# codeMonkey339/Congestion-control-with-BitTorren

Hardware: AMD Instinct MI355X
Metric: GiB/s device-resident SHA-1 over 512KB chunks; % of HBM-read roofline (higher is better)
Workload: dtype u32; 1 GPU; 4096 x 524288 B chunks per GPU, device-resident (BASELINE config 2); chunks_per_gpu=4096, chunk_bytes=524288, kernel=split_u4_2prod, kernel_requested=auto, streams=1, parallelism=chunk-sharded x1, no collective

## Files before the change

congestion-control-with-bittorren_amd/csrc/sha1_kernels.h:

```cpp
#pragma once

#include <hip/hip_runtime.h>
#include <stdint.h>

struct BatchArgs {
    const uint8_t* base;
    const uint64_t* off;
    const uint32_t* len;
    uint32_t ulen;
    uint32_t n;
    const uint32_t* order;
    uint8_t* dig;
    const uint32_t* init_state;
    uint64_t prefix_bytes;
    uint32_t* out_state;
    const uint32_t* plan;
};

enum LaunchCounter {
    kLaunchLane, kLaunchFused, kLaunchSplit1, kLaunchSplit4, kLaunchSplit11Lane, kLaunchSplit11Shared,
    kLaunchQuad, kLaunchStudy, kLaunchMixed, kLaunchSort, kLaunchDrain, kLaunchCounters
};
void count_launch(LaunchCounter which);

hipError_t launch_lane(const BatchArgs& A, hipStream_t st);
hipError_t launch_fused(const BatchArgs& A, hipStream_t st);
constexpr int kSplitUnitQuad = 416;
bool split_unit_built(int unit_blocks);
hipError_t launch_split(const BatchArgs& A, int unit_blocks, hipStream_t st);
bool split_unit_study_built(int unit_blocks);
hipError_t launch_split_study(const BatchArgs& A, int unit_blocks, hipStream_t st);
uint32_t mixed_grid(uint32_t groups, int cus, uint32_t* hcap);
constexpr uint32_t kBigExact = 4096;
struct BigFix {
    const uint32_t* cnt;
    uint32_t tiles;
    const uint32_t* len;
    const uint32_t* id;
    uint32_t* order;
    uint32_t* sorted_len;
};
hipError_t launch_mixed(const BatchArgs& A, const uint32_t* sorted_len, const BigFix* big, uint32_t* plan, int cus,
                        const int* forced, hipStream_t st);
hipError_t launch_plan_layout(const BatchArgs& A, const uint32_t* sorted_len, const BigFix* big, uint32_t* plan,
                              hipStream_t st);
struct VqDrainArgs {
    const uint8_t* data;
    const uint64_t* off;
    const uint32_t* len;
    const uint8_t* exp;
    const uint32_t* grp;
    const uint32_t* pub;
    const uint32_t* stop;
    uint8_t* alive;
    uint8_t* res;
    uint32_t* done;
    uint32_t* last_done;
    uint8_t* dig;
    uint32_t* claim;
    uint32_t grp_ring;
    uint32_t pad;
    uint64_t idle_ticks;
    uint64_t life_ticks;
};
hipError_t launch_vq_drain(const VqDrainArgs& Q, uint32_t grid, hipStream_t st);

struct PvEntry {
    uint32_t session;
    uint32_t from;
    uint32_t upto;
    uint32_t len;
    uint32_t final;
    uint32_t gen;
    uint32_t pad[2];
};
struct PvArgs {
    const uint8_t* data;
    uint64_t stride;
    const PvEntry* work;
    uint32_t n;
    uint32_t sessions;
    uint32_t* state;
    const uint32_t* expected;
    uint32_t* result;
    uint32_t* done;
    const uint8_t* dummy;
};
hipError_t launch_progress(const PvArgs& P, int depth, hipStream_t st);
hipError_t launch_progress_shared(const PvArgs& P, hipStream_t st);

struct UpdateArgs {
    uint8_t* ctx;
    uint64_t n_contexts;
    const uint32_t* index;
    uint32_t n;
    const uint8_t* base;
    const uint64_t* off;
    const uint32_t* len;
    uint64_t* mid_off;
    uint32_t* mid_len;
    uint32_t* state;
    uint8_t* dig;
};
hipError_t launch_update_init(const UpdateArgs& U, hipStream_t st);
hipError_t launch_update_pre(const UpdateArgs& U, hipStream_t st);
hipError_t launch_update_post(const UpdateArgs& U, hipStream_t st);
hipError_t launch_update_final(const UpdateArgs& U, hipStream_t st);

struct GatherArgs {
    const uint8_t* base;
// ... 44 lines not shown
```

congestion-control-with-bittorren_amd/csrc/sha1_kernels.hip:

```cpp
#include <hip/hip_runtime.h>
#include <stdint.h>

#include <algorithm>
#include <cstdlib>
#include <cstring>

#include "sha1_fused.hpp"
#include "sha1_split.hpp"

#define PLAN_SPLIT4 0.743
#define PLAN_SPLIT8 0.860
#define PLAN_FUSED4T 1.254
#define PLAN_FUSED4S 1.334
#define PLAN_FUSED8T 2.502
#define PLAN_FUSED8S 2.628
#define PLAN_FUSED_SHARE 0.955

__global__ __launch_bounds__(256) void sha1_lane_kernel(BatchArgs A) {
    const uint32_t e = blockIdx.x * blockDim.x + threadIdx.x;
    if (e >= A.n) return;
    const Entry en = fetch_entry(A, e);
    uint32_t h[5];
    load_init(A, en.id, h);
    lane_blocks(A, en, 0, h);
// ... 781 lines not shown
        for (uint32_t m = 32; m >= 1; m >>= 1) key = min(key, (uint64_t)__shfl_xor(key, m));
        if (lane == 0u) red[wv] = key;
    }
    __syncthreads();
    if (t == 0) {
        ts[5] = __builtin_amdgcn_s_memrealtime();
        cs[5] = __builtin_amdgcn_s_memtime();
        uint64_t key = red[0];
#pragma unroll
        for (uint32_t w = 1; w < kMaxCand / 64; ++w) key = min(key, red[w]);
        uint32_t bi = (uint32_t)key;
        if (cmk[2] <= cmk[bi] * 1.005f) bi = 2;
        plan[0] = cmode[bi];
        plan[1] = cmode[bi] == 1 ? 0u : chead[bi];
        plan[2] = cmode[bi] == 1 ? 0u : cf[bi];
#pragma unroll
        for (int i = 1; i < 6; ++i) plan[7 + i] = static_cast<uint32_t>(ts[i] - ts[0]);
#pragma unroll
        for (int i = 1; i < 6; ++i) plan[13 + i] = static_cast<uint32_t>(cs[i] - cs[0]);
#pragma unroll
        for (int i = 0; i < 3; ++i) plan[20 + i] = static_cast<uint32_t>(sub[i] - cs[0]);
        plan[23] = nrun;
#pragma unroll
        for (int i = 0; i < 3; ++i) plan[24 + i] = static_cast<uint32_t>(bsub[i] - cs[0]);
        plan[27] = simcyc;
    }
}

__device__ __forceinline__ uint64_t splitmix64(uint64_t x) {
    uint64_t z = x + 0x9E3779B97F4A7C15ull;
    z = (z ^ (z >> 30)) * 0xBF58476D1CE4E5B9ull;
    z = (z ^ (z >> 27)) * 0x94D049BB133111EBull;
    return z ^ (z >> 31);
}

__global__ __launch_bounds__(kSynthThreads) void synth_fill_kernel(uint8_t* dst, const uint64_t* off,
                                                         const uint32_t* lens, uint32_t ulen,
                                                         uint64_t first, uint64_t seed) {
    const uint64_t c = blockIdx.x;
    const uint32_t len = lens ? lens[c] : ulen;
    uint8_t* out = dst + (off ? off[c] : c * (uint64_t)ulen);
    const uint64_t key = seed ^ ((first + c) << 24);
    const uint32_t nw = len >> 3;
    uint64_t* o = reinterpret_cast<uint64_t*>(out);
    for (uint32_t w = threadIdx.x; w < nw; w += blockDim.x) o[w] = splitmix64(key ^ (uint64_t)w);
    const uint32_t rem = len & 7u;
    if (rem && threadIdx.x == 0) {
        const uint64_t v = splitmix64(key ^ (uint64_t)nw);
        for (uint32_t b = 0; b < rem; ++b) out[8ull * nw + b] = (uint8_t)(v >> (8 * b));
    }
}

__global__ __launch_bounds__(256) void compare_kernel(const uint8_t* dig, const uint8_t* exp,
                                                      uint32_t n, uint8_t* mismatch) {
    const uint32_t i = blockIdx.x * blockDim.x + threadIdx.x;
    if (i >= n) return;
    uint32_t diff = 0;
#pragma unroll
    for (int b = 0; b < 20; ++b) diff |= (uint32_t)(dig[20ull * i + b] ^ exp[20ull * i + b]);
    mismatch[i] = diff ? 1 : 0;
}

hipError_t launch_lane(const BatchArgs& A, hipStream_t st) {
    if (A.n == 0) return hipSuccess;
    const uint32_t grid = (A.n + 255u) / 256u;
    count_launch(kLaunchLane);
    hipLaunchKernelGGL(sha1_lane_kernel, dim3(grid), dim3(256), 0, st, A);
    return hipGetLastError();
}

hipError_t launch_fused(const BatchArgs& A, hipStream_t st) {
    if (A.n == 0) return hipSuccess;
    count_launch(kLaunchFused);
    hipLaunchKernelGGL(sha1_fused_kernel, dim3((A.n + 255u) / 256u), dim3(256), 0, st, A);
    return hipGetLastError();
}

__attribute__((weak)) bool split_unit_study_built(int) { return false; }
__attribute__((weak)) hipError_t launch_split_study(const BatchArgs&, int, hipStream_t) {
    return hipErrorInvalidValue;
}

bool split_unit_built(int u) {
    return u == 1 || u == 4 || u == 11 || u == kSplitUnitQuad || split_unit_study_built(u);
}

static_assert(kSplitThreads<1, kSplitV<1>, 1> == 128, "unit 1: consumer + producer");
static_assert(kSplitThreads<1, kSplitV<4>, kSplitNProd<4>> == 256, "unit 4: consumer, two producers, wave 2 empty");
static_assert(kSplitThreads<2, kSplit8V, 2> == 512 && kSplitThreads<2, kSplit8V & ~kVCoop, 2> == 512,
              "unit 11: the 8-wave layout");
static_assert(kSplitThreads<1, kSplitQuadV, 2> == 256, "unit 416: as unit 4");

hipError_t launch_split(const BatchArgs& A, int unit_blocks, hipStream_t st) {
    if (A.n == 0) return hipSuccess;
    const uint32_t groups = (A.n + 63u) / 64u;
    switch (unit_blocks) {
    case 1:
        count_launch(kLaunchSplit1);
        launch_shape<1, 1>(A, groups, st);
        break;
    case 4:
        count_launch(kLaunchSplit4);
        launch_shape<4, 1, kSplitV<4>, kSplitNProd<4>>(A, groups, st);
        break;
    case 11:
        if (A.off == nullptr && A.order == nullptr) {
            count_launch(kLaunchSplit11Lane);
            launch_shape<2, 2, kSplit8V & ~kVCoop, 2>(A, (groups + 1) / 2, st);
        } else {
            count_launch(kLaunchSplit11Shared);
            launch_shape<2, 2, kSplit8V, 2>(A, (groups + 1) / 2, st);
        }
        break;
    case kSplitUnitQuad:
        count_launch(kLaunchQuad);
        launch_shape<4, 1, kSplitQuadV, 2>(A, (A.n + 15u) / 16u, st);
        break;
    default: return launch_split_study(A, unit_blocks, st);
    }
    return hipGetLastError();
}

uint32_t mixed_grid(uint32_t groups, int cus, uint32_t* hcap) {
    *hcap = std::min<uint32_t>(std::min<uint32_t>(groups, 4u * (uint32_t)cus), kPlanMaxH);
    return groups;
}

hipError_t launch_plan_layout(const BatchArgs& A, const uint32_t* sorted_len, const BigFix* big, uint32_t* plan,
                              hipStream_t st) {
    if (A.n == 0) return hipSuccess;
    const uint32_t groups = (A.n + 63u) / 64u;
    const uint32_t words = (groups + 31u) / 32u;
    uint64_t* lay_tb = reinterpret_cast<uint64_t*>(plan + 64);
    uint32_t* lay_bits = reinterpret_cast<uint32_t*>(lay_tb + words);
    uint32_t* lay_blk = lay_bits + words;
    hipLaunchKernelGGL(plan_layout_kernel, dim3(words), dim3(kLayoutThreads), 0, st, A, sorted_len,
                       big ? *big : BigFix{}, lay_tb, lay_bits, lay_blk);
    return hipGetLastError();
}

hipError_t launch_mixed(const BatchArgs& A, const uint32_t* sorted_len, const BigFix* big, uint32_t* plan, int cus,
                        const int* forced, hipStream_t st) {
    if (A.n == 0) return hipSuccess;
    const uint32_t groups = (A.n + 63u) / 64u;
    uint32_t hcap;
    const uint32_t grid = mixed_grid(groups, cus, &hcap);
    const uint32_t words = (groups + 31u) / 32u;
    uint64_t* lay_tb = reinterpret_cast<uint64_t*>(plan + 64);
    uint32_t* lay_bits = reinterpret_cast<uint32_t*>(lay_tb + words);
    const uint32_t* lay_blk = lay_bits + words;
    count_launch(kLaunchMixed);
    if (!forced) {
        const hipError_t le = launch_plan_layout(A, sorted_len, big, plan, st);
        if (le != hipSuccess) return le;
    }
    hipLaunchKernelGGL(plan_mixed_kernel, dim3(1), dim3(kPlanThreads), 0, st, A, sorted_len,
                       (uint32_t)cus, hcap, forced ? 1 : 0, forced ? (uint32_t)forced[0] : 0u,
                       forced ? (uint32_t)forced[1] : 0u, forced ? (uint32_t)forced[2] : 0u, plan, lay_tb,
                       lay_bits, lay_blk);
    hipError_t e = hipGetLastError();
    if (e != hipSuccess) return e;
    BatchArgs B = A;
    B.plan = plan;
    const char* disp = getenv("SHA1CHUNK_MIXED_DISPATCH");
    const bool persistent = !(disp && !strcmp(disp, "hw"));
    if (persistent)
        hipLaunchKernelGGL(sha1_mixed_persistent_kernel, dim3((uint32_t)cus), dim3(kMixedThreads), 0, st, B,
                           plan + 3);
    else
        hipLaunchKernelGGL(sha1_mixed_kernel, dim3(grid), dim3(kMixedThreads), 0, st, B);
    return hipGetLastError();
}

hipError_t launch_vq_drain(const VqDrainArgs& Q, uint32_t grid, hipStream_t st) {
    count_launch(kLaunchDrain);
    hipLaunchKernelGGL(sha1_vq_drain_kernel, dim3(grid), dim3(kMixedThreads), 0, st, Q);
    return hipGetLastError();
}

hipError_t launch_synth(uint8_t* dst, const uint64_t* off, const uint32_t* lens, uint32_t ulen,
                        uint64_t first, uint64_t count, uint64_t seed, hipStream_t st) {
    if (count == 0) return hipSuccess;
    if (count > kSynthMaxChunks) return hipErrorInvalidValue;
    hipLaunchKernelGGL(synth_fill_kernel, dim3((uint32_t)count), dim3(kSynthThreads), 0, st, dst, off, lens,
                       ulen, first, seed);
    return hipGetLastError();
}

hipError_t launch_compare(const uint8_t* dig, const uint8_t* exp, uint32_t n, uint8_t* mismatch,
                          hipStream_t st) {
    if (n == 0) return hipSuccess;
    hipLaunchKernelGGL(compare_kernel, dim3((n + 255u) / 256u), dim3(256), 0, st, dig, exp, n,
                       mismatch);
    return hipGetLastError();
}

#ifdef SHA1CHUNK_CHECKED
extern "C" __attribute__((visibility("default"))) long long s1be_checked_violations(int reset) {
    int cur = 0, nd = 0;
    if (hipGetDevice(&cur) != hipSuccess || hipGetDeviceCount(&nd) != hipSuccess) return -1;
// ... 17 lines not shown
```

congestion-control-with-bittorren_amd/csrc/sha1_runtime.hip:

```cpp
#include <algorithm>
#include <cstdio>
#include <cstdlib>
#include <cstring>
#include <mutex>
#include <numeric>
#include <string>
#include <thread>
#include <vector>

#include "sha1_runtime_internal.h"

using namespace s1rt;

namespace {
int split_unit(size_t n, int cus) {
    if (const char* e = getenv("SHA1CHUNK_SPLIT_UNIT")) return atoi(e);
    if ((n + 15) / 16 <= size_t(std::max(0, cus - drain_cus_held()))) return kSplitUnitQuad;
    const size_t groups = (n + 63) / 64;
    if (groups <= size_t(cus)) return 4;
    if (groups <= size_t(cus) * 2) return 11;
    return 1;
}

hipError_t launch(int kernel, const BatchArgs& A, int cus, hipStream_t st) {
    switch (kernel) {
    case SHA1CHUNK_KERNEL_LANE: return launch_lane(A, st);
    case SHA1CHUNK_KERNEL_FUSED: return launch_fused(A, st);
    case SHA1CHUNK_KERNEL_SPLIT: return launch_split(A, split_unit(A.n, cus), st);
    default: return hipErrorInvalidValue;
    }
}

int check_batch(const BatchArgs& A) {
    if (A.n > 0xffffffffu - 1024u)
        return fail(SHA1CHUNK_EINVAL, "batch of %u chunks: at most 2^32 - 1025 per call", A.n);
    if (A.n > 0 && (reinterpret_cast<uintptr_t>(A.dig) & 3u))
        return fail(SHA1CHUNK_EALIGN, "digest buffer must be 4-byte aligned");
    return SHA1CHUNK_OK;
}
}

namespace s1rt {
int choose_kernel(int kernel, size_t n, int cus) {
    if (kernel != SHA1CHUNK_KERNEL_AUTO) return kernel;
    if (const char* f = getenv("SHA1CHUNK_FORCE_KERNEL")) {
        if (!strcmp(f, "lane")) return SHA1CHUNK_KERNEL_LANE;
        if (!strcmp(f, "fused")) return SHA1CHUNK_KERNEL_FUSED;
        if (!strcmp(f, "split")) return SHA1CHUNK_KERNEL_SPLIT;
    }
    const size_t groups = (n + 63) / 64;
    return groups <= size_t(cus) * 2 ? SHA1CHUNK_KERNEL_SPLIT : SHA1CHUNK_KERNEL_FUSED;
}

int launch_checked(int kernel, const BatchArgs& A, hipStream_t st, int cus) {
    if (kernel < SHA1CHUNK_KERNEL_LANE || kernel > SHA1CHUNK_KERNEL_SPLIT)
        return fail(SHA1CHUNK_EINVAL, "unknown kernel id %d", kernel);
    if (int rc = check_batch(A)) return rc;
    if (kernel == SHA1CHUNK_KERNEL_SPLIT && !split_unit_built(split_unit(A.n, cus)))
        return fail(SHA1CHUNK_EINVAL, "split shape %d is not in this library (A/B shapes: `make ab`)",
                    split_unit(A.n, cus));
    hipError_t e = launch(kernel, A, cus, st);
    if (e != hipSuccess) return fail(SHA1CHUNK_EHIP, "kernel launch: %s", hipGetErrorString(e));
    return SHA1CHUNK_OK;
}

bool use_mixed(size_t n, int cus) {
    if (getenv("SHA1CHUNK_FORCE_KERNEL")) return false;
    const char* e = getenv("SHA1CHUNK_MIXED");
    if (e && !strcmp(e, "0")) return false;
    if (e && !strcmp(e, "all")) return true;
    return (n + 63) / 64 > size_t(cus);
}

int launch_mixed_checked(const BatchArgs& A, const uint32_t* sorted_len, const BigFix* big, uint32_t* plan, int cus,
                         hipStream_t st) {
    if (int rc = check_batch(A)) return rc;
    int forced[3] = {0, 0, 0};
    bool force = false;
    if (const char* e = getenv("SHA1CHUNK_MIXED_PLAN")) {
        uint32_t hcap;
        const uint32_t groups = (A.n + 63u) / 64u;
        (void)mixed_grid(groups, cus, &hcap);
        if (sscanf(e, "%d,%d,%d", &forced[0], &forced[1], &forced[2]) != 3 || forced[0] < 0 ||
            forced[0] > 1 ||
            (forced[0] == 0 && (forced[1] < 0 || ((uint32_t)forced[1] > hcap && (uint32_t)forced[1] != groups) ||
                                (forced[2] != 4 && forced[2] != 8))))
            return fail(SHA1CHUNK_EINVAL,
                        "SHA1CHUNK_MIXED_PLAN=%s: want 0,H,F (0 <= H <= %u or H = %u, F 4|8) or 1,0,0", e,
                        hcap, groups);
        force = true;
    }
    hipError_t e = launch_mixed(A, sorted_len, big, plan, cus, force ? forced : nullptr, st);
    if (e != hipSuccess) return fail(SHA1CHUNK_EHIP, "mixed kernel launch: %s", hipGetErrorString(e));
    if (const char* d = getenv("SHA1CHUNK_MIXED_DEBUG"); d && atoi(d)) {
        uint32_t p[28];
        HIP_TRY(hipMemcpyAsync(p, plan, sizeof p, hipMemcpyDeviceToHost, st));
        HIP_TRY(hipStreamSynchronize(st));
        fprintf(stderr, "sha1chunk mixed plan: n=%u groups=%u cus=%d mode=%u H=%u F=%u\n", A.n,
                (A.n + 63u) / 64u, cus, p[0], p[1], p[2]);
        if (!force && p[12])
            fprintf(stderr,
                    "sha1chunk mixed planner stages: scan %.1f bounds %.1f sweep %.1f pass2 %.1f pass3 %.1f us;"
// ... 470 lines not shown
```

congestion-control-with-bittorren_amd/csrc/sha1_split.hpp:

```cpp
#ifndef SHA1_SPLIT_HPP
#define SHA1_SPLIT_HPP

#include "sha1_lane.hpp"

constexpr int kWBlockBytes = 20 * 1024;

constexpr int kVWK = 1;
constexpr int kVUnmask = 4;
constexpr int kVRead10 = 8;
constexpr int kVSkipWave2 = 64;
constexpr int kVLayout8 = 128;
constexpr int kVCross = 256;
constexpr int kVProbe = 2048;
constexpr int kVCoop = 8192;
constexpr int kVQuad = 8192 * 4;

template <int U>
constexpr int kSplitV = U == 4 ? (kVWK | kVUnmask | kVSkipWave2 | kVRead10 | kVCoop)
                               : U == 3 ? kVUnmask : (kVWK | kVUnmask);
template <int U>
constexpr int kSplitNProd = U == 4 ? 2 : 1;
constexpr int kSplit8V = kVWK | kVUnmask | kVLayout8 | kVCross | kVCoop;
constexpr int kSplitQuadV = kVWK | kVUnmask | kVSkipWave2 | kVCoop | kVQuad;
template <int PAIRS, int V, int NPROD>
constexpr int kSplitThreads = (V & kVLayout8) ? 512 : 64 * PAIRS * (1 + NPROD) + ((V & kVSkipWave2) ? 64 : 0);


__device__ __forceinline__ void split_barrier() {
    __builtin_amdgcn_s_waitcnt(0xC07F);
    asm volatile("s_barrier" ::: "memory");
}

__device__ __forceinline__ void split_barrier_timed(uint64_t& acc) {
    __builtin_amdgcn_s_waitcnt(0xC07F);
    const uint64_t t0 = __builtin_amdgcn_s_memtime();
    asm volatile("s_barrier" ::: "memory");
    acc += __builtin_amdgcn_s_memtime() - t0;
}

template <int T, bool WK>
struct SchedWrite {
    __device__ __forceinline__ static void run(uint32_t (&w)[16], uint8_t* slot, int lane) {
        if constexpr (T < 80) {
            if constexpr (T >= 16) sched_step<T>(w);
            if constexpr ((T & 3) == 3) {
                constexpr int j = (T - 3) & 15;
                constexpr uint32_t k = WK ? round_k<T>() : 0u;
                *reinterpret_cast<uint4*>(slot + (T >> 2) * 1024 + lane * 16) =
                    make_uint4(w[j] + k, w[j + 1] + k, w[j + 2] + k, w[j + 3] + k);
            }
            SchedWrite<T + 1, WK>::run(w, slot, lane);
        }
    }
};

__device__ __forceinline__ uint32_t total_blocks(uint32_t len) {
    return (len >> 6) + (((len & 63u) < 56u) ? 1u : 2u);
}

__device__ __forceinline__ void tail_block_words(const Entry& en, uint32_t k, uint32_t (&w)[16]) {
    const uint32_t nfull = en.len >> 6, rem = en.len & 63u;
    const uint64_t bits = (uint64_t)en.len * 8ull;
    if (k < nfull) {
        load_block16(en.p + 64ull * k, w);
#pragma unroll
        for (int j = 0; j < 16; ++j) w[j] = bswap(w[j]);
    } else if (k == nfull) {
        if (rem) {
            load_block_partial(en.p + 64ull * k, rem, w);
        } else {
#pragma unroll
            for (int j = 0; j < 16; ++j) w[j] = 0u;
        }
#pragma unroll
        for (int j = 0; j < 16; ++j) w[j] = pad_word(bswap(w[j]), j, (int)rem);
        if (rem < 56u) {
            w[14] = (uint32_t)(bits >> 32);
            w[15] = (uint32_t)bits;
        }
    } else {
#pragma unroll
        for (int j = 0; j < 14; ++j) w[j] = 0u;
        w[14] = (uint32_t)(bits >> 32);
        w[15] = (uint32_t)bits;
    }
}

template <int U, bool WK, int NPROD = 1>
__device__ __forceinline__ void produce_block(uint32_t k, uint32_t (&w)[16], uint8_t* ring, int lane,
                                              uint64_t* bw = nullptr) {
    const uint32_t m = k / U, j = k - m * U;
    SchedWrite<0, WK>::run(w, ring + ((m & 1u) * U + j) * kWBlockBytes, lane);
    if (NPROD == 1 ? j == U - 1 : (U == NPROD || (k & 1u) == 1u)) {
        if (bw)
            split_barrier_timed(*bw);
        else
            split_barrier();
    }
}


template <int U, bool WK, int NPROD = 1>
__device__ __forceinline__ void produce_stage(const Entry& en, uint32_t s, uint32_t S, Stage& cur,
                                              uint8_t* ring, int lane) {
#pragma unroll
    for (int half = 0; half < 2; ++half) {
// ... 70 lines not shown
template <bool MASK>
__device__ __forceinline__ void commit(uint32_t (&h)[5], const uint32_t (&v)[5], bool live) {
    if constexpr (MASK) {
#pragma unroll
        for (int i = 0; i < 5; ++i) h[i] = live ? h[i] + v[i] : h[i];
    } else {
#pragma unroll
        for (int i = 0; i < 5; ++i) h[i] += v[i];
    }
}

__device__ __forceinline__ void probe_store(const BatchArgs& A, uint32_t row, uint64_t waited, uint64_t total,
                                            uint32_t blocks) {
    uint32_t* o = reinterpret_cast<uint32_t*>(A.dig + 20ull * row);
    o[0] = (uint32_t)waited;
    o[1] = (uint32_t)(waited >> 32);
    o[2] = (uint32_t)total;
    o[3] = (uint32_t)(total >> 32);
    o[4] = blocks;
}

template <int B, int NB, bool WK>
struct BurstRounds {
    __device__ __forceinline__ static void run(uint32_t (&v)[5], const uint32_t (&Wc)[80], uint32_t (&Wn)[80],
                                               const uint8_t* slot) {
        if constexpr (B < NB) {
            __builtin_amdgcn_sched_barrier(0);
            read_w_groups<4 * B / NB, 4 * (B + 1) / NB>(slot, Wn);
            __builtin_amdgcn_sched_barrier(0);
            RoundsW<80 * B / NB, 80 * (B + 1) / NB, WK>::run(v, Wc);
            BurstRounds<B + 1, NB, WK>::run(v, Wc, Wn, slot);
        }
    }
};

template <int U, int J, int V, bool MASK>
__device__ __forceinline__ void consume_block(uint32_t k, uint32_t T, uint32_t (&h)[5],
                                              const uint32_t (&Wc)[80], uint32_t (&Wn)[80],
                                              const uint8_t* ring, int lane, uint64_t& bw) {
    constexpr int jn = (J + 1) % U;
    constexpr int slot_idx = (((J + 1) / U) & 1) * U + jn;
    const uint8_t* slot = ring + slot_idx * kWBlockBytes + lane * 16;
    uint32_t v[5] = {h[0], h[1], h[2], h[3], h[4]};
    if constexpr (jn == 0) split_barrier_or_timed<V>(bw);
    BurstRounds<0, (V & kVRead10) ? 2 : 4, (V & kVWK) != 0>::run(v, Wc, Wn, slot);
    commit<MASK>(h, v, k < T);
}

template <int U, int J, int V, bool MASK>
struct ConsumeUnits {
    __device__ __forceinline__ static void run(uint32_t k0, uint32_t T, uint32_t (&h)[5],
                                               uint32_t (&Wa)[80], uint32_t (&Wb)[80],
                                               const uint8_t* ring, int lane, uint64_t& bw) {
        if constexpr (J < 2 * U) {
            consume_block<U, J, V, MASK>(k0 + J, T, h, Wa, Wb, ring, lane, bw);
            ConsumeUnits<U, J + 1, V, MASK>::run(k0, T, h, Wb, Wa, ring, lane, bw);
        }
    }
};

template <int U, int V>
__device__ __forceinline__ void consume_all(const BatchArgs& A, const Entry& en, bool valid, uint32_t T,
                                            uint32_t units, const uint8_t* ring, int lane) {
    uint32_t h[5];
    load_init(A, en.id, h);
    uint32_t Wa[80], Wb[80];
    split_barrier();
    read_w_groups<0, 4>(ring + lane * 16, Wa);
    const uint32_t Tmin = __builtin_amdgcn_readfirstlane(wave_min(valid ? T : 0xffffffffu));
    const uint32_t full = (V & kVUnmask) ? min(Tmin, units * U) / (2 * U) * (2 * U) : 0u;
    uint32_t k = 0;
    uint64_t bw = 0;
    const uint64_t t0 = (V & kVProbe) ? __builtin_amdgcn_s_memtime() : 0;
    for (; k < full; k += 2 * U) ConsumeUnits<U, 0, V, false>::run(k, T, h, Wa, Wb, ring, lane, bw);
    for (; k < units * U; k += 2 * U) ConsumeUnits<U, 0, V, true>::run(k, T, h, Wa, Wb, ring, lane, bw);
    if constexpr ((V & kVProbe) != 0) {
        const uint64_t tot = __builtin_amdgcn_s_memtime() - t0;
        if (lane == 0) probe_store(A, en.id & ~63u, bw, tot, units * U);
        return;
    }
    if (valid) emit(A, en.id, h);
}

constexpr int kQuadBlockBytes = 5 * 1024;

template <int SEL>
__device__ __forceinline__ uint32_t quad_bcast(uint32_t x) {
    return (uint32_t)__builtin_amdgcn_update_dpp(0, (int)x, SEL * 0x55, 0xf, 0xf, true);
}

__device__ __forceinline__ void quad_align() { asm volatile(".p2align 3"); }

template <int T, int END>
struct RoundsQ {
    __device__ __forceinline__ static void run(uint32_t (&v)[5], const uint32_t (&W)[20]) {
        if constexpr (T < END) {
            round_step<T, true, true>(v, quad_bcast<(T >> 2) & 3>(W[4 * (T >> 4) + (T & 3)]));
            RoundsQ<T + 1, END>::run(v, W);
        }
    }
};

__device__ __forceinline__ void quad_read_w(const uint8_t* slot, uint32_t (&W)[20]) {
#pragma unroll
    for (int q = 0; q < 5; ++q) unpack4(W + 4 * q, *reinterpret_cast<const uint4*>(slot + q * 1024));
}

template <int U, int J, int V, bool MASK>
__device__ __forceinline__ void quad_consume_block(uint32_t k, uint32_t T, uint32_t (&h)[5],
                                                   const uint32_t (&Wc)[20], uint32_t (&Wn)[20],
                                                   const uint8_t* ring, int lane, uint64_t& bw) {
    constexpr int jn = (J + 1) % U;
    constexpr int slot_idx = (((J + 1) / U) & 1) * U + jn;
    const uint8_t* slot = ring + slot_idx * kQuadBlockBytes + lane * 16;
    uint32_t v[5] = {h[0], h[1], h[2], h[3], h[4]};
    if constexpr (jn == 0) split_barrier_or_timed<V>(bw);
    __builtin_amdgcn_sched_barrier(0);
    quad_read_w(slot, Wn);
    __builtin_amdgcn_sched_barrier(0);
    quad_align();
    __builtin_amdgcn_sched_barrier(0);
    RoundsQ<0, 80>::run(v, Wc);
    __builtin_amdgcn_sched_barrier(0);
    __builtin_amdgcn_s_waitcnt(0xC07F);
    __builtin_amdgcn_sched_barrier(0);
    commit<MASK>(h, v, k < T);
    __builtin_amdgcn_sched_barrier(0);
}

template <int U, int J, int V, bool MASK>
struct QuadConsumeUnits {
    __device__ __forceinline__ static void run(uint32_t k0, uint32_t T, uint32_t (&h)[5], uint32_t (&Wa)[20],
                                               uint32_t (&Wb)[20], const uint8_t* ring, int lane, uint64_t& bw) {
        if constexpr (J < 2 * U) {
            quad_consume_block<U, J, V, MASK>(k0 + J, T, h, Wa, Wb, ring, lane, bw);
            QuadConsumeUnits<U, J + 1, V, MASK>::run(k0, T, h, Wb, Wa, ring, lane, bw);
        }
    }
};

template <int T>
struct QuadSchedWrite {
    __device__ __forceinline__ static void run(uint32_t (&w)[16], uint8_t* slot, bool j1, bool j2,
                                               const uint32_t (&kq)[5]) {
        if constexpr (T < 80) {
            if constexpr (T >= 16) sched_step<T>(w);
            if constexpr ((T & 15) == 15) {
                constexpr int q = T >> 4;
                uint32_t o[4];
#pragma unroll
                for (int i = 0; i < 4; ++i) {
                    const uint32_t lo = j1 ? w[4 + i] : w[i], hi = j1 ? w[12 + i] : w[8 + i];
                    o[i] = (j2 ? hi : lo) + kq[q];
                }
                *reinterpret_cast<uint4*>(slot + q * 1024) = make_uint4(o[0], o[1], o[2], o[3]);
            }
            QuadSchedWrite<T + 1>::run(w, slot, j1, j2, kq);
        }
    }
};

template <int U>
__device__ __forceinline__ void quad_produce_block(uint32_t k, uint32_t (&w)[16], uint8_t* ring, int lane,
                                                   const uint32_t (&kq)[5]) {
    const uint32_t m = k / U, j = k - m * U;
    QuadSchedWrite<0>::run(w, ring + ((m & 1u) * U + j) * kQuadBlockBytes + lane * 16, (lane & 1) != 0,
                           (lane & 2) != 0, kq);
    if ((k & 1u) == 1u && ((k >> 1) % (U / 2)) + 2 >= U / 2) split_barrier();
}

__device__ __forceinline__ void quad_block_words(const uint32_t (&x)[4], uint32_t (&w)[16]) {
    uint32_t y[4];
#pragma unroll
    for (int i = 0; i < 4; ++i) y[i] = bswap(x[i]);
#pragma unroll
    for (int i = 0; i < 4; ++i) {
        w[i] = quad_bcast<0>(y[i]);
        w[4 + i] = quad_bcast<1>(y[i]);
        w[8 + i] = quad_bcast<2>(y[i]);
        w[12 + i] = quad_bcast<3>(y[i]);
    }
}

__device__ __forceinline__ void quad_load_stage(const u32x4u* src, uint32_t s, uint32_t (&x)[8]) {
#pragma unroll
    for (int b = 0; b < 2; ++b) unpack4(x + 4 * b, src[8u * s + 4u * b]);
}

template <int U>
__device__ __forceinline__ void quad_produce_stage(const u32x4u* src, uint32_t s, uint32_t S, uint32_t (&cur)[8],
                                                   uint8_t* ring, int lane, const uint32_t (&kq)[5]) {
    uint32_t x0[4] = {cur[0], cur[1], cur[2], cur[3]}, x1[4] = {cur[4], cur[5], cur[6], cur[7]};
    if (s + 4 < S) quad_load_stage(src, s + 4, cur);
    uint32_t w[16];
    quad_block_words(x0, w);
    quad_produce_block<U>(2 * s, w, ring, lane, kq);
    quad_block_words(x1, w);
    quad_produce_block<U>(2 * s + 1, w, ring, lane, kq);
}

template <int U, int V>
__device__ __forceinline__ void quad_consume_all(const BatchArgs& A, const Entry& en, bool valid, uint32_t T,
                                                 uint32_t units, const uint8_t* ring, int lane, uint32_t wg) {
    uint32_t h[5];
    load_init(A, en.id, h);
    uint32_t Wa[20], Wb[20];
    split_barrier();
    quad_read_w(ring + lane * 16, Wa);
    __builtin_amdgcn_s_waitcnt(0x0070);
    const uint32_t Tmin = __builtin_amdgcn_readfirstlane(wave_min(valid ? T : 0xffffffffu));
    const uint32_t full = min(Tmin, units * U) / (2 * U) * (2 * U);
    uint32_t k = 0;
    uint64_t bw = 0;
    const uint64_t t0 = (V & kVProbe) ? __builtin_amdgcn_s_memtime() : 0;
    for (; k < full; k += 2 * U) QuadConsumeUnits<U, 0, V, false>::run(k, T, h, Wa, Wb, ring, lane, bw);
    for (; k < units * U; k += 2 * U) QuadConsumeUnits<U, 0, V, true>::run(k, T, h, Wa, Wb, ring, lane, bw);
    if constexpr ((V & kVProbe) != 0) {
        const uint64_t tot = __builtin_amdgcn_s_memtime() - t0;
        if (lane == 0) probe_store(A, wg * 16u, bw, tot, units * U);
        return;
    }
    if (valid && (lane & 3) == 0) emit(A, en.id, h);
}

template <int U, int V, int NPROD>
__device__ __forceinline__ void quad_split_body(const BatchArgs& A, uint8_t* ring, uint32_t wg) {
    static_assert((U == 4 || U == 8) && NPROD == 2 && (V & kVSkipWave2) != 0 && (V & kVWK) != 0 &&
                      (V & kVUnmask) != 0,
                  "quad shape: 4- or 8-block units, two producers on waves 1 and 3, W+K shipped");
    int wave = __builtin_amdgcn_readfirstlane(threadIdx.x >> 6);
    if (wave == 2) return;
    const bool producer = wave != 0;
    const uint32_t pidx = wave == 3 ? 1u : 0u;
    const int lane = threadIdx.x & 63;
    bool valid;
    const Entry en = lane_entry(A, wg * 16u + ((uint32_t)lane >> 2), min(wg * 16u, A.n - 1u), valid);
    const uint32_t T = valid ? (A.out_state ? (en.len >> 6) : total_blocks(en.len)) : 0u;
    const uint32_t Tmax = __builtin_amdgcn_readfirstlane(wave_max(T));
    const uint32_t units = (Tmax + 2 * U - 1) / (2 * U) * 2;
    if (!producer) {
        quad_consume_all<U, V>(A, en, valid, T, units, ring, lane, wg);
        return;
    }
    uint32_t kq[5];
#pragma unroll
    for (int q = 0; q < 5; ++q) {
        const uint32_t t = 16u * q + 4u * ((uint32_t)lane & 3u);
        kq[q] = t < 20 ? K0 : t < 40 ? K1 : t < 60 ? K2 : K3;
    }
    const uint32_t S = bulk_stages(en, valid);
    const u32x4u* src = reinterpret_cast<const u32x4u*>(en.p) + (lane & 3);
    uint32_t C0[8], C1[8];
    uint32_t s = pidx;
    if (s < S) quad_load_stage(src, s, C0);
    if (s + 2 < S) quad_load_stage(src, s + 2, C1);
    for (; s + 2 < S; s += 4) {
        quad_produce_stage<U>(src, s, S, C0, ring, lane, kq);
        quad_produce_stage<U>(src, s + 2, S, C1, ring, lane, kq);
    }
    if (s < S) {
        quad_produce_stage<U>(src, s, S, C0, ring, lane, kq);
        s += 2;
    }
    for (; 2 * s < units * U; s += 2) {
#pragma unroll
        for (int half = 0; half < 2; ++half) {
            const uint32_t k = 2 * s + half;
            uint32_t w[16];
            if (k < T) tail_block_words(en, k, w);
            quad_produce_block<U>(k, w, ring, lane, kq);
        }
    }
    split_barrier();
}

template <int U, int PAIRS, int V, int NPROD>
__device__ __forceinline__ void split_body(const BatchArgs& A, uint8_t* lds, uint32_t wg) {
    if constexpr ((V & kVQuad) != 0) {
        static_assert(PAIRS == 1, "quad shape: one consumer per workgroup");
        quad_split_body<U, V, NPROD>(A, lds, wg);
        return;
    }
    constexpr bool WK = (V & kVWK) != 0;
    static_assert((V & kVQuad) != 0 || PAIRS * 2 * U * kWBlockBytes <= 160 * 1024, "LDS");
    static_assert((V & kVQuad) != 0 || NPROD == 1 || (PAIRS == 1 && (U == 2 * NPROD || U == NPROD)) ||
                      (PAIRS == 2 && U == NPROD && (V & kVLayout8) != 0),
                  "two producers: one stage (U = 4) or one block (U = 2, 8-wave layout) each per unit");
    int wave = __builtin_amdgcn_readfirstlane(threadIdx.x >> 6);
    if constexpr ((V & kVSkipWave2) != 0) {
        static_assert(NPROD == 2 && PAIRS == 1, "skip-wave layout is for two producers");
        if (wave == 2) return;
        if (wave > 2) wave -= 1;
    }
    int pair = wave % PAIRS;
    bool producer = wave >= PAIRS;
    uint32_t pidx = producer ? (uint32_t)(wave - PAIRS) / PAIRS : 0u;
    if constexpr ((V & kVLayout8) != 0) {
        static_assert(PAIRS == 2 && NPROD == 2, "8-wave layout: two pairs, two producers each");
        if (wave == 4 || wave == 6) return;
        producer = (wave & 1) != 0;
        pair = producer ? (((wave >> 1) & 1) ^ ((V & kVCross) ? 1 : 0)) : (wave >> 1);
        pidx = producer ? (uint32_t)(wave >> 2) : 0u;
    }
    const int lane = threadIdx.x & 63;
    uint8_t* ring = lds + pair * (2 * U * kWBlockBytes);
    const uint32_t group = wg * PAIRS + (uint32_t)pair;
    bool valid;
    const Entry en = lane_entry(A, group * 64u + (uint32_t)lane, fallback_entry(A, group), valid);
    const uint32_t T = valid ? (A.out_state ? (en.len >> 6) : total_blocks(en.len)) : 0u;
    uint32_t Tmax = __builtin_amdgcn_readfirstlane(wave_max(T));
    if constexpr (PAIRS > 1) {
        uint32_t* slots = reinterpret_cast<uint32_t*>(lds);
        if (!producer && lane == 0) slots[pair] = Tmax;
        __syncthreads();
#pragma unroll
        for (int q = 0; q < PAIRS; ++q) Tmax = max(Tmax, slots[q]);
        Tmax = __builtin_amdgcn_readfirstlane(Tmax);
        __syncthreads();
    }
    const uint32_t units = (Tmax + 2 * U - 1) / (2 * U) * 2;

    if (producer) {
        const uint32_t S = bulk_stages(en, valid);
        if constexpr (U == NPROD) {
            const uint32_t K = S * 2u;
            uint32_t B0[16], B1[16];
            uint32_t k = pidx;
            uint64_t pbw = 0;
            uint64_t* const pb = (V & kVProbe) ? &pbw : nullptr;
            const uint64_t pt0 = (V & kVProbe) ? __builtin_amdgcn_s_memtime() : 0;
            if constexpr ((V & kVCoop) != 0) {
                const u32x4u* src[4];
                coop_sources<4>(A, group, (uint32_t)lane, src);
                if (pidx < K) coop4_load(src, pidx, B0);
                if (pidx + NPROD < K) coop4_load(src, pidx + NPROD, B1);
                for (; k + NPROD < K; k += 2 * NPROD) {
                    produce_own_block_coop<U, WK, NPROD>(src, k, K, B0, ring, (uint32_t)lane, pb);
                    produce_own_block_coop<U, WK, NPROD>(src, k + NPROD, K, B1, ring, (uint32_t)lane, pb);
                }
                if (k < K) {
                    produce_own_block_coop<U, WK, NPROD>(src, k, K, B0, ring, (uint32_t)lane, pb);
                    k += NPROD;
                }
            } else {
                if (pidx < K) load_block16(en.p + 64ull * pidx, B0);
                if (pidx + NPROD < K) load_block16(en.p + 64ull * (pidx + NPROD), B1);
                for (; k + NPROD < K; k += 2 * NPROD) {
                    produce_own_block<U, WK, NPROD>(en, k, K, B0, ring, lane, pb);
                    produce_own_block<U, WK, NPROD>(en, k + NPROD, K, B1, ring, lane, pb);
                }
                if (k < K) {
                    produce_own_block<U, WK, NPROD>(en, k, K, B0, ring, lane, pb);
                    k += NPROD;
                }
            }
            for (; k < units * U; k += NPROD) {
                uint32_t w[16];
                if (k < T) tail_block_words(en, k, w);
                produce_block<U, WK, NPROD>(k, w, ring, lane, pb);
            }
            if constexpr ((V & kVProbe) != 0) {
                const uint64_t tot = __builtin_amdgcn_s_memtime() - pt0;
                if (lane == 0) probe_store(A, group * 64u + 1u + pidx, pbw, tot, units * U);
            }
            split_barrier();
            return;
        }
        uint32_t s = pidx;
        if constexpr ((V & kVCoop) != 0) {
            const u32x4u* src[8];
            coop_sources<8>(A, group, (uint32_t)lane, src);
            uint32_t C0[32], C1[32];
            if (pidx < S) coop_load(src, pidx, C0);
            if (pidx + NPROD < S) coop_load(src, pidx + NPROD, C1);
            for (; s + NPROD < S; s += 2 * NPROD) {
                produce_stage_coop<U, WK, NPROD>(src, s, S, C0, ring, (uint32_t)lane);
                produce_stage_coop<U, WK, NPROD>(src, s + NPROD, S, C1, ring, (uint32_t)lane);
            }
            if (s < S) {
                produce_stage_coop<U, WK, NPROD>(src, s, S, C0, ring, (uint32_t)lane);
                s += NPROD;
            }
        } else {
            Stage A0, A1;
            if (pidx < S) load_stage(en.p + 128ull * pidx, A0);
            if (pidx + NPROD < S) load_stage(en.p + 128ull * (pidx + NPROD), A1);
            for (; s + NPROD < S; s += 2 * NPROD) {
                produce_stage<U, WK, NPROD>(en, s, S, A0, ring, lane);
                produce_stage<U, WK, NPROD>(en, s + NPROD, S, A1, ring, lane);
            }
            if (s < S) {
                produce_stage<U, WK, NPROD>(en, s, S, A0, ring, lane);
                s += NPROD;
            }
        }
        for (; 2 * s < units * U; s += NPROD) {
#pragma unroll
            for (int half = 0; half < 2; ++half) {
                const uint32_t k = 2 * s + half;
                uint32_t w[16];
                if (k < T) tail_block_words(en, k, w);
                produce_block<U, WK, NPROD>(k, w, ring, lane);
            }
        }
        split_barrier();
    } else {
        consume_all<U, V>(A, en, valid, T, units, ring, lane);
    }
}

template <int U, int PAIRS, int V>
constexpr int kSplitLdsBytes = (V & kVQuad) ? 2 * U * kQuadBlockBytes : PAIRS * 2 * U * kWBlockBytes;

template <int U, int PAIRS, int V = kSplitV<U>, int NPROD = 1>
__global__ __launch_bounds__((kSplitThreads<PAIRS, V, NPROD>)) void sha1_split_kernel(
    BatchArgs A) {
    __shared__ __attribute__((aligned(16))) uint8_t lds[kSplitLdsBytes<U, PAIRS, V>];
    split_body<U, PAIRS, V, NPROD>(A, lds, blockIdx.x);
}

template <int U, int PAIRS, int V = kSplitV<U>, int NPROD = 1>
void launch_shape(const BatchArgs& A, uint32_t grid, hipStream_t st) {
    hipLaunchKernelGGL((sha1_split_kernel<U, PAIRS, V, NPROD>), dim3(grid), dim3(kSplitThreads<PAIRS, V, NPROD>), 0,
                       st, A);
}

#endif
```

Baseline: 344.6 GiB/s.

## Add pair-lane split kernel hashing each chunk across two lanes

Adds a new split kernel shape (unit 432) where each chunk is processed by two lanes instead of four (quad) or one. This gives 32 chunks per workgroup, with DPP broadcasts and a 10 KiB-per-block LDS ring. The runtime selects it when the chunk groups fit in the CUs and n/32 fits in the free CUs. The aim is more parallelism per chunk than the single-lane unit 4 path, giving finer latency hiding without the quad shape's per-lane overhead. In exchange it uses more LDS per block and more cross-lane broadcast work per round.

```diff
diff --git a/congestion-control-with-bittorren_amd/csrc/sha1_kernels.h b/congestion-control-with-bittorren_amd/csrc/sha1_kernels.h
--- a/congestion-control-with-bittorren_amd/csrc/sha1_kernels.h
+++ b/congestion-control-with-bittorren_amd/csrc/sha1_kernels.h
@@ -26,6 +26,7 @@
 hipError_t launch_lane(const BatchArgs& A, hipStream_t st);
 hipError_t launch_fused(const BatchArgs& A, hipStream_t st);
 constexpr int kSplitUnitQuad = 416;
+constexpr int kSplitUnitPair = 432;
 bool split_unit_built(int unit_blocks);
 hipError_t launch_split(const BatchArgs& A, int unit_blocks, hipStream_t st);
 bool split_unit_study_built(int unit_blocks);
diff --git a/congestion-control-with-bittorren_amd/csrc/sha1_kernels.hip b/congestion-control-with-bittorren_amd/csrc/sha1_kernels.hip
--- a/congestion-control-with-bittorren_amd/csrc/sha1_kernels.hip
+++ b/congestion-control-with-bittorren_amd/csrc/sha1_kernels.hip
@@ -887,7 +887,7 @@
 }
 
 bool split_unit_built(int u) {
-    return u == 1 || u == 4 || u == 11 || u == kSplitUnitQuad || split_unit_study_built(u);
+    return u == 1 || u == 4 || u == 11 || u == kSplitUnitQuad || u == kSplitUnitPair || split_unit_study_built(u);
 }
 
 static_assert(kSplitThreads<1, kSplitV<1>, 1> == 128, "unit 1: consumer + producer");
@@ -895,6 +895,8 @@
 static_assert(kSplitThreads<2, kSplit8V, 2> == 512 && kSplitThreads<2, kSplit8V & ~kVCoop, 2> == 512,
               "unit 11: the 8-wave layout");
 static_assert(kSplitThreads<1, kSplitQuadV, 2> == 256, "unit 416: as unit 4");
+static_assert(kSplitThreads<1, kSplitPairV, 2> == 256, "unit 432: as unit 4");
+static_assert(kSplitLdsBytes<4, 1, kSplitPairV> == 80 * 1024, "unit 432: 2 x 4 x 10 KiB of LDS");
 
 hipError_t launch_split(const BatchArgs& A, int unit_blocks, hipStream_t st) {
     if (A.n == 0) return hipSuccess;
@@ -921,6 +923,10 @@
         count_launch(kLaunchQuad);
         launch_shape<4, 1, kSplitQuadV, 2>(A, (A.n + 15u) / 16u, st);
         break;
+    case kSplitUnitPair:
+        count_launch(kLaunchSplit4);
+        launch_shape<4, 1, kSplitPairV, 2>(A, (A.n + 31u) / 32u, st);
+        break;
     default: return launch_split_study(A, unit_blocks, st);
     }
     return hipGetLastError();
diff --git a/congestion-control-with-bittorren_amd/csrc/sha1_runtime.hip b/congestion-control-with-bittorren_amd/csrc/sha1_runtime.hip
--- a/congestion-control-with-bittorren_amd/csrc/sha1_runtime.hip
+++ b/congestion-control-with-bittorren_amd/csrc/sha1_runtime.hip
@@ -15,9 +15,10 @@
 namespace {
 int split_unit(size_t n, int cus) {
     if (const char* e = getenv("SHA1CHUNK_SPLIT_UNIT")) return atoi(e);
-    if ((n + 15) / 16 <= size_t(std::max(0, cus - drain_cus_held()))) return kSplitUnitQuad;
+    const size_t free_cus = size_t(std::max(0, cus - drain_cus_held()));
+    if ((n + 15) / 16 <= free_cus) return kSplitUnitQuad;
     const size_t groups = (n + 63) / 64;
-    if (groups <= size_t(cus)) return 4;
+    if (groups <= size_t(cus)) return (n + 31) / 32 <= free_cus ? kSplitUnitPair : 4;
     if (groups <= size_t(cus) * 2) return 11;
     return 1;
 }
diff --git a/congestion-control-with-bittorren_amd/csrc/sha1_split.hpp b/congestion-control-with-bittorren_amd/csrc/sha1_split.hpp
--- a/congestion-control-with-bittorren_amd/csrc/sha1_split.hpp
+++ b/congestion-control-with-bittorren_amd/csrc/sha1_split.hpp
@@ -14,6 +14,7 @@
 constexpr int kVProbe = 2048;
 constexpr int kVCoop = 8192;
 constexpr int kVQuad = 8192 * 4;
+constexpr int kVPair = 8192 * 8;
 
 template <int U>
 constexpr int kSplitV = U == 4 ? (kVWK | kVUnmask | kVSkipWave2 | kVRead10 | kVCoop)
@@ -22,6 +23,9 @@
 constexpr int kSplitNProd = U == 4 ? 2 : 1;
 constexpr int kSplit8V = kVWK | kVUnmask | kVLayout8 | kVCross | kVCoop;
 constexpr int kSplitQuadV = kVWK | kVUnmask | kVSkipWave2 | kVCoop | kVQuad;
+constexpr int kSplitPairV = kVWK | kVUnmask | kVSkipWave2 | kVCoop | kVPair;
+template <int V>
+constexpr int kChunkLanes = (V & kVQuad) ? 4 : (V & kVPair) ? 2 : 1;
 template <int PAIRS, int V, int NPROD>
 constexpr int kSplitThreads = (V & kVLayout8) ? 512 : 64 * PAIRS * (1 + NPROD) + ((V & kVSkipWave2) ? 64 : 0);
 
@@ -258,37 +262,50 @@
     if (valid) emit(A, en.id, h);
 }
 
-constexpr int kQuadBlockBytes = 5 * 1024;
-
-template <int SEL>
+template <int L>
+constexpr int kLanesBlockBytes = 20 * 1024 / L;
+constexpr int kQuadBlockBytes = kLanesBlockBytes<4>;
+constexpr int kPairBlockBytes = kLanesBlockBytes<2>;
+
+template <int SEL, int L = 4>
 __device__ __forceinline__ uint32_t quad_bcast(uint32_t x) {
-    return (uint32_t)__builtin_amdgcn_update_dpp(0, (int)x, SEL * 0x55, 0xf, 0xf, true);
+    static_assert((L == 4 && SEL < 4) || (L == 2 && SEL < 2), "lane of the chunk");
+    constexpr int ctrl = L == 4 ? SEL * 0x55 : SEL * 0x55 + 0xA0;
+    return (uint32_t)__builtin_amdgcn_update_dpp(0, (int)x, ctrl, 0xf, 0xf, true);
 }
 
 __device__ __forceinline__ void quad_align() { asm volatile(".p2align 3"); }
 
-template <int T, int END>
+template <int T, int END, int L = 4>
 struct RoundsQ {
-    __device__ __forceinline__ static void run(uint32_t (&v)[5], const uint32_t (&W)[20]) {
+    __device__ __forceinline__ static void run(uint32_t (&v)[5], const uint32_t (&W)[80 / L]) {
         if constexpr (T < END) {
-            round_step<T, true, true>(v, quad_bcast<(T >> 2) & 3>(W[4 * (T >> 4) + (T & 3)]));
-            RoundsQ<T + 1, END>::run(v, W);
+            round_step<T, true, true>(v, quad_bcast<(T >> 2) % L, L>(W[4 * (T / (4 * L)) + (T & 3)]));
+            RoundsQ<T + 1, END, L>::run(v, W);
         }
     }
 };
 
-__device__ __forceinline__ void quad_read_w(const uint8_t* slot, uint32_t (&W)[20]) {
-#pragma unroll
-    for (int q = 0; q < 5; ++q) unpack4(W + 4 * q, *reinterpret_cast<const uint4*>(slot + q * 1024));
+template <int NW>
+__device__ __forceinline__ void quad_read_w(const uint8_t* slot, uint32_t (&W)[NW]) {
+#pragma unroll
+    for (int q = 0; q < NW / 4; ++q) unpack4(W + 4 * q, *reinterpret_cast<const uint4*>(slot + q * 1024));
 }
 
 template <int U, int J, int V, bool MASK>
 __device__ __forceinline__ void quad_consume_block(uint32_t k, uint32_t T, uint32_t (&h)[5],
-                                                   const uint32_t (&Wc)[20], uint32_t (&Wn)[20],
+                                                   const uint32_t (&Wc)[80 / kChunkLanes<V>],
+                                                   uint32_t (&Wn)[80 / kChunkLanes<V>],
                                                    const uint8_t* ring, int lane, uint64_t& bw) {
+    constexpr int L = kChunkLanes<V>;
     constexpr int jn = (J + 1) % U;
     constexpr int slot_idx = (((J + 1) / U) & 1) * U + jn;
-    const uint8_t* slot = ring + slot_idx * kQuadBlockBytes + lane * 16;
+    const uint8_t* slot = ring + slot_idx * kLanesBlockBytes<L> + lane * 16;
+    if constexpr (L == 2 && slot_idx >= U) {
+        int hi = lane * 16 + U * kLanesBlockBytes<L>;
+        asm("" : "+v"(hi));
+        slot = ring + (slot_idx - U) * kLanesBlockBytes<L> + hi;
+    }
     uint32_t v[5] = {h[0], h[1], h[2], h[3], h[4]};
     if constexpr (jn == 0) split_barrier_or_timed<V>(bw);
     __builtin_amdgcn_sched_barrier(0);
@@ -296,7 +313,7 @@
     __builtin_amdgcn_sched_barrier(0);
     quad_align();
     __builtin_amdgcn_sched_barrier(0);
-    RoundsQ<0, 80>::run(v, Wc);
+    RoundsQ<0, 80, L>::run(v, Wc);
     __builtin_amdgcn_sched_barrier(0);
     __builtin_amdgcn_s_waitcnt(0xC07F);
     __builtin_amdgcn_sched_barrier(0);
@@ -306,8 +323,10 @@
 
 template <int U, int J, int V, bool MASK>
 struct QuadConsumeUnits {
-    __device__ __forceinline__ static void run(uint32_t k0, uint32_t T, uint32_t (&h)[5], uint32_t (&Wa)[20],
-                                               uint32_t (&Wb)[20], const uint8_t* ring, int lane, uint64_t& bw) {
+    __device__ __forceinline__ static void run(uint32_t k0, uint32_t T, uint32_t (&h)[5],
+                                               uint32_t (&Wa)[80 / kChunkLanes<V>],
+                                               uint32_t (&Wb)[80 / kChunkLanes<V>], const uint8_t* ring, int lane,
+                                               uint64_t& bw) {
         if constexpr (J < 2 * U) {
             quad_consume_block<U, J, V, MASK>(k0 + J, T, h, Wa, Wb, ring, lane, bw);
             QuadConsumeUnits<U, J + 1, V, MASK>::run(k0, T, h, Wb, Wa, ring, lane, bw);
@@ -315,33 +334,39 @@
     }
 };
 
-template <int T>
+template <int T, int L = 4>
 struct QuadSchedWrite {
     __device__ __forceinline__ static void run(uint32_t (&w)[16], uint8_t* slot, bool j1, bool j2,
-                                               const uint32_t (&kq)[5]) {
+                                               const uint32_t (&kq)[20 / L]) {
         if constexpr (T < 80) {
             if constexpr (T >= 16) sched_step<T>(w);
-            if constexpr ((T & 15) == 15) {
-                constexpr int q = T >> 4;
+            if constexpr ((T & (4 * L - 1)) == 4 * L - 1) {
+                constexpr int q = T / (4 * L);
                 uint32_t o[4];
-#pragma unroll
-                for (int i = 0; i < 4; ++i) {
-                    const uint32_t lo = j1 ? w[4 + i] : w[i], hi = j1 ? w[12 + i] : w[8 + i];
-                    o[i] = (j2 ? hi : lo) + kq[q];
+                if constexpr (L == 4) {
+#pragma unroll
+                    for (int i = 0; i < 4; ++i) {
+                        const uint32_t lo = j1 ? w[4 + i] : w[i], hi = j1 ? w[12 + i] : w[8 + i];
+                        o[i] = (j2 ? hi : lo) + kq[q];
+                    }
+                } else {
+                    constexpr int base = 8 * (q & 1);
+#pragma unroll
+                    for (int i = 0; i < 4; ++i) o[i] = (j1 ? w[base + 4 + i] : w[base + i]) + kq[q];
                 }
                 *reinterpret_cast<uint4*>(slot + q * 1024) = make_uint4(o[0], o[1], o[2], o[3]);
             }
-            QuadSchedWrite<T + 1>::run(w, slot, j1, j2, kq);
+            QuadSchedWrite<T + 1, L>::run(w, slot, j1, j2, kq);
         }
     }
 };
 
-template <int U>
+template <int U, int L = 4>
 __device__ __forceinline__ void quad_produce_block(uint32_t k, uint32_t (&w)[16], uint8_t* ring, int lane,
-                                                   const uint32_t (&kq)[5]) {
+                                                   const uint32_t (&kq)[20 / L]) {
     const uint32_t m = k / U, j = k - m * U;
-    QuadSchedWrite<0>::run(w, ring + ((m & 1u) * U + j) * kQuadBlockBytes + lane * 16, (lane & 1) != 0,
-                           (lane & 2) != 0, kq);
+    QuadSchedWrite<0, L>::run(w, ring + ((m & 1u) * U + j) * kLanesBlockBytes<L> + lane * 16, (lane & 1) != 0,
+                              (lane & 2) != 0, kq);
     if ((k & 1u) == 1u && ((k >> 1) % (U / 2)) + 2 >= U / 2) split_barrier();
 }
 
@@ -358,9 +383,26 @@
     }
 }
 
+__device__ __forceinline__ void quad_block_words(const uint32_t (&x)[8], uint32_t (&w)[16]) {
+    uint32_t y[8];
+#pragma unroll
+    for (int i = 0; i < 8; ++i) y[i] = bswap(x[i]);
+#pragma unroll
+    for (int i = 0; i < 4; ++i) {
+        w[i] = quad_bcast<0, 2>(y[i]);
+        w[4 + i] = quad_bcast<1, 2>(y[i]);
+        w[8 + i] = quad_bcast<0, 2>(y[4 + i]);
+        w[12 + i] = quad_bcast<1, 2>(y[4 + i]);
+    }
+}
+
 __device__ __forceinline__ void quad_load_stage(const u32x4u* src, uint32_t s, uint32_t (&x)[8]) {
 #pragma unroll
     for (int b = 0; b < 2; ++b) unpack4(x + 4 * b, src[8u * s + 4u * b]);
+}
+__device__ __forceinline__ void quad_load_stage(const u32x4u* src, uint32_t s, uint32_t (&x)[16]) {
+#pragma unroll
+    for (int p = 0; p < 4; ++p) unpack4(x + 4 * p, src[8u * s + 2u * p]);
 }
 
 template <int U>
@@ -374,13 +416,30 @@
     quad_block_words(x1, w);
     quad_produce_block<U>(2 * s + 1, w, ring, lane, kq);
 }
+template <int U>
+__device__ __forceinline__ void quad_produce_stage(const u32x4u* src, uint32_t s, uint32_t S, uint32_t (&cur)[16],
+                                                   uint8_t* ring, int lane, const uint32_t (&kq)[10]) {
+    uint32_t x0[8], x1[8];
+#pragma unroll
+    for (int i = 0; i < 8; ++i) {
+        x0[i] = cur[i];
+        x1[i] = cur[8 + i];
+    }
+    if (s + 4 < S) quad_load_stage(src, s + 4, cur);
+    uint32_t w[16];
+    quad_block_words(x0, w);
+    quad_produce_block<U, 2>(2 * s, w, ring, lane, kq);
+    quad_block_words(x1, w);
+    quad_produce_block<U, 2>(2 * s + 1, w, ring, lane, kq);
+}
 
 template <int U, int V>
 __device__ __forceinline__ void quad_consume_all(const BatchArgs& A, const Entry& en, bool valid, uint32_t T,
                                                  uint32_t units, const uint8_t* ring, int lane, uint32_t wg) {
     uint32_t h[5];
     load_init(A, en.id, h);
-    uint32_t Wa[20], Wb[20];
+    constexpr int L = kChunkLanes<V>;
+    uint32_t Wa[80 / L], Wb[80 / L];
     split_barrier();
     quad_read_w(ring + lane * 16, Wa);
     __builtin_amdgcn_s_waitcnt(0x0070);
@@ -393,24 +452,26 @@
     for (; k < units * U; k += 2 * U) QuadConsumeUnits<U, 0, V, true>::run(k, T, h, Wa, Wb, ring, lane, bw);
     if constexpr ((V & kVProbe) != 0) {
         const uint64_t tot = __builtin_amdgcn_s_memtime() - t0;
-        if (lane == 0) probe_store(A, wg * 16u, bw, tot, units * U);
+        if (lane == 0) probe_store(A, wg * (64u / L), bw, tot, units * U);
         return;
     }
-    if (valid && (lane & 3) == 0) emit(A, en.id, h);
+    if (valid && (lane & (L - 1)) == 0) emit(A, en.id, h);
 }
 
 template <int U, int V, int NPROD>
 __device__ __forceinline__ void quad_split_body(const BatchArgs& A, uint8_t* ring, uint32_t wg) {
-    static_assert((U == 4 || U == 8) && NPROD == 2 && (V & kVSkipWave2) != 0 && (V & kVWK) != 0 &&
-                      (V & kVUnmask) != 0,
-                  "quad shape: 4- or 8-block units, two producers on waves 1 and 3, W+K shipped");
+    constexpr int L = kChunkLanes<V>;
+    constexpr uint32_t CPW = 64u / L;
+    static_assert((U == 4 || (U == 8 && L == 4)) && NPROD == 2 && (V & kVSkipWave2) != 0 && (V & kVWK) != 0 &&
+                      (V & kVUnmask) != 0 && (L == 2 || L == 4) && !((V & kVQuad) != 0 && (V & kVPair) != 0),
+                  "quad shape: 4- or 8-block units, two producers on waves 1 and 3, W+K shipped; pair: 4-block");
     int wave = __builtin_amdgcn_readfirstlane(threadIdx.x >> 6);
     if (wave == 2) return;
     const bool producer = wave != 0;
     const uint32_t pidx = wave == 3 ? 1u : 0u;
     const int lane = threadIdx.x & 63;
     bool valid;
-    const Entry en = lane_entry(A, wg * 16u + ((uint32_t)lane >> 2), min(wg * 16u, A.n - 1u), valid);
+    const Entry en = lane_entry(A, wg * CPW + ((uint32_t)lane / L), min(wg * CPW, A.n - 1u), valid);
     const uint32_t T = valid ? (A.out_state ? (en.len >> 6) : total_blocks(en.len)) : 0u;
     const uint32_t Tmax = __builtin_amdgcn_readfirstlane(wave_max(T));
     const uint32_t units = (Tmax + 2 * U - 1) / (2 * U) * 2;
@@ -418,15 +479,15 @@
         quad_consume_all<U, V>(A, en, valid, T, units, ring, lane, wg);
         return;
     }
-    uint32_t kq[5];
-#pragma unroll
-    for (int q = 0; q < 5; ++q) {
-        const uint32_t t = 16u * q + 4u * ((uint32_t)lane & 3u);
+    uint32_t kq[20 / L];
+#pragma unroll
+    for (int q = 0; q < 20 / L; ++q) {
+        const uint32_t t = 4u * L * q + 4u * ((uint32_t)lane & (L - 1u));
         kq[q] = t < 20 ? K0 : t < 40 ? K1 : t < 60 ? K2 : K3;
     }
     const uint32_t S = bulk_stages(en, valid);
-    const u32x4u* src = reinterpret_cast<const u32x4u*>(en.p) + (lane & 3);
-    uint32_t C0[8], C1[8];
+    const u32x4u* src = reinterpret_cast<const u32x4u*>(en.p) + (lane & (L - 1));
+    uint32_t C0[32 / L], C1[32 / L];
     uint32_t s = pidx;
     if (s < S) quad_load_stage(src, s, C0);
     if (s + 2 < S) quad_load_stage(src, s + 2, C1);
@@ -444,7 +505,7 @@
             const uint32_t k = 2 * s + half;
             uint32_t w[16];
             if (k < T) tail_block_words(en, k, w);
-            quad_produce_block<U>(k, w, ring, lane, kq);
+            quad_produce_block<U, L>(k, w, ring, lane, kq);
         }
     }
     split_barrier();
@@ -452,8 +513,8 @@
 
 template <int U, int PAIRS, int V, int NPROD>
 __device__ __forceinline__ void split_body(const BatchArgs& A, uint8_t* lds, uint32_t wg) {
-    if constexpr ((V & kVQuad) != 0) {
-        static_assert(PAIRS == 1, "quad shape: one consumer per workgroup");
+    if constexpr ((V & (kVQuad | kVPair)) != 0) {
+        static_assert(PAIRS == 1, "quad and pair shapes: one consumer per workgroup");
         quad_split_body<U, V, NPROD>(A, lds, wg);
         return;
     }
@@ -586,7 +647,9 @@
 }
 
 template <int U, int PAIRS, int V>
-constexpr int kSplitLdsBytes = (V & kVQuad) ? 2 * U * kQuadBlockBytes : PAIRS * 2 * U * kWBlockBytes;
+constexpr int kSplitLdsBytes = (V & kVQuad)   ? 2 * U * kQuadBlockBytes
+                               : (V & kVPair) ? 2 * U * kPairBlockBytes
+                                              : PAIRS * 2 * U * kWBlockBytes;
 
 template <int U, int PAIRS, int V = kSplitV<U>, int NPROD = 1>
 __global__ __launch_bounds__((kSplitThreads<PAIRS, V, NPROD>)) void sha1_split_kernel(
```

Result: no change. 344.6 GiB/s, median of 2 (+0.0%).
